# chiy48308/audio_feature_extraction

Measured on AMD Instinct MI355X. Metric: audio frames/sec (sr=22050, n_fft=1024, hop=256, n_mfcc=13), higher is better.
Workload: dtype f32; 1 GPU; 1000x10s clips @22050 Hz per GPU, frame_length=1024, hop_length=256, n_mfcc=13, n_mels=128, hamming, pre-emphasis 0.97 + trim 30 dB + RMS (BASELINE configs[1]); clips_per_gpu=1000, frames_per_gpu_step=862000, input=HBM-resident float32

## Files before the change

### audio_feature_extraction_amd/csrc/afx_api.cpp

```cpp
#include <algorithm>
#include <cmath>
#include <cstdio>
#include <cstdlib>
#include <cstring>
#include <atomic>
#include <mutex>
#include <string>
#include <vector>

#include <hip/hip_runtime.h>

#include "afx_device.h"
#include "afx_devenv.h"
#include "afx_frames3.h"
#include "afx_internal.h"
#include "afx_plan.h"

namespace afx {
DevEnv::DevEnv() {
  if (const char* v = getenv("AFX_DEBUG_SKIP")) debug_skip = atoi(v) & 127;
  if (const char* v = getenv("AFX_F0_DEBUG")) f0_debug = atoi(v);
  stamps = getenv("AFX_DEBUG_STAMPS") != nullptr;
  f3_debug = getenv("AFX_F3_DEBUG") != nullptr;
  no_spec = getenv("AFX_NO_SPEC") != nullptr;
  no_tickets = getenv("AFX_NO_TICKETS") != nullptr;
  no_frames3 = getenv("AFX_NO_FRAMES3") != nullptr;
  no_frames3s = getenv("AFX_NO_FRAMES3S") != nullptr;
  no_frames3d = getenv("AFX_NO_FRAMES3D") != nullptr;
  f3_generic_mel = getenv("AFX_F3_GENERIC_MEL") != nullptr;
  no_dct16l = getenv("AFX_NO_DCT16L") != nullptr;
  host_blocks = getenv("AFX_HOST_BLOCKS") != nullptr;
  no_fused_tail = getenv("AFX_NO_FUSED_TAIL") != nullptr;
  if (const char* v = getenv("AFX_F3_WAVES")) f3_waves = atoi(v);
  if (const char* v = getenv("AFX_F3_SPARE_CUS")) f3_spare_cus = atoi(v) < 0 ? -2 : atoi(v);
  if (const char* v = getenv("AFX_TAIL_MODE")) tail_mode = atoi(v);
  if (const char* v = getenv("AFX_TAIL_SKIP")) tail_skip = atoi(v) & 7;
  if (const char* v = getenv("AFX_TEST_CHUNK_CLIPS")) chunk_clips = std::max(1, std::min(32768, atoi(v)));
  if (const char* v = getenv("AFX_TEST_F0_CHUNK_FRAMES")) f0_chunk_frames = std::max<int64_t>(64, atoll(v));
  if (const char* v = getenv("AFX_TEST_DTW_BUDGET")) dtw_budget = std::max<int64_t>(1, atoll(v));
  if (const char* v = getenv("AFX_TEST_HPSS_BUDGET")) hpss_budget = std::max<int64_t>(1, atoll(v));
  if (const char* v = getenv("AFX_TEST_CHROMA_BUDGET")) chroma_budget = std::max<int64_t>(1, atoll(v));
  if (const char* v = getenv("AFX_TEST_RHYTHM_BUDGET")) rhythm_budget = std::max<int64_t>(1, atoll(v));
  if (const char* v = getenv("AFX_TEST_GROUPS_BUDGET")) groups_budget = std::max<int64_t>(1, atoll(v));
  if (const char* v = getenv("AFX_TEST_FILT_BUDGET")) filt_budget = std::max<int64_t>(1, atoll(v));
  f0_dump = getenv("AFX_F0_DUMP");
}
const DevEnv& dev_env() { static const DevEnv e; return e; }
}

extern "C" int afx_device_count(void) {
  int n = 0;
  if (hipGetDeviceCount(&n) != hipSuccess) return 0;
  return n;
}

extern "C" int afx_init(int device, afx_ctx** out) {
  if (!out) { set_error("afx_init: null out"); return AFX_ERR_INVALID; }
  *out = nullptr;
  int n = afx_device_count();
  if (n <= 0) { set_error("no HIP device visible"); return AFX_ERR_NO_DEVICE; }
  if (device < 0 || device >= n) { set_error("device index out of range"); return AFX_ERR_INVALID; }
  HIP_TRY(hipSetDevice(device));
  afx_ctx* c = new afx_ctx();
  c->device = device;
  hipError_t e = hipStreamCreateWithFlags(&c->stream, hipStreamNonBlocking);
  if (e != hipSuccess) { delete c; set_error(std::string("hipStreamCreate: ") + hipGetErrorString(e)); return AFX_ERR_HIP; }
  *out = c;
  return AFX_OK;
}

extern "C" void afx_destroy(afx_ctx* ctx) {
  if (!ctx) return;
  (void)hipSetDevice(ctx->device);
  for (DevBuf* b : {&ctx->dtw_raw, &ctx->dtw_feats, &ctx->dtw_norms, &ctx->dtw_pairs, &ctx->dtw_codes, &ctx->dtw_rows, &ctx->dtw_d,
                    &ctx->dtw_path, &ctx->dtw_cost, &ctx->dtw_status, &ctx->dtw_len, &ctx->dtw_end, &ctx->rs_g, &ctx->rs_tstart, &ctx->rs_clips,
                    &ctx->rs_in, &ctx->rs_out, &ctx->dc_clips, &ctx->dc_in, &ctx->dc_out, &ctx->ft_tab, &ctx->ft_clips, &ctx->ft_st,
                    &ctx->ft_w, &ctx->ft_carry, &ctx->ft_tmax, &ctx->ft_in, &ctx->ft_out})
    release(*b);
  if (ctx->stream) (void)hipStreamDestroy(ctx->stream);
  delete ctx;
}

extern "C" int afx_malloc(afx_ctx* ctx, size_t bytes, void** out) {
  if (!ctx || !out) { set_error("afx_malloc: null argument"); return AFX_ERR_INVALID; }
  HIP_TRY(hipSetDevice(ctx->device));
  hipError_t e = hipMalloc(out, bytes ? bytes : 1);
  if (e != hipSuccess) { set_error(std::string("hipMalloc: ") + hipGetErrorString(e)); return e == hipErrorOutOfMemory ? AFX_ERR_NOMEM : AFX_ERR_HIP; }
  return AFX_OK;
}

extern "C" int afx_free(afx_ctx* ctx, void* d) {
  if (!ctx) { set_error("afx_free: null ctx"); return AFX_ERR_INVALID; }
  HIP_TRY(hipSetDevice(ctx->device));
  if (d) HIP_TRY(hipFree(d));
  return AFX_OK;
}

extern "C" int afx_host_alloc(afx_ctx* ctx, size_t bytes, void** out) {
  if (!ctx || !out) { set_error("afx_host_alloc: null argument"); return AFX_ERR_INVALID; }
  *out = nullptr;
  HIP_TRY(hipSetDevice(ctx->device));
  hipError_t e = hipHostMalloc(out, bytes ? bytes : 1, hipHostMallocPortable);
  if (e != hipSuccess) { set_error(std::string("hipHostMalloc: ") + hipGetErrorString(e)); *out = nullptr; return e == hipErrorOutOfMemory ? AFX_ERR_NOMEM : AFX_ERR_HIP; }
  return AFX_OK;
}

extern "C" int afx_host_free(afx_ctx* ctx, void* h) {
  if (!ctx) { set_error("afx_host_free: null ctx"); return AFX_ERR_INVALID; }
  HIP_TRY(hipSetDevice(ctx->device));
  if (h) HIP_TRY(hipHostFree(h));
  return AFX_OK;
}

extern "C" int afx_memcpy_h2d(afx_ctx* ctx, void* dst, const void* src, size_t bytes) {
  if (!ctx || (!dst && bytes) || (!src && bytes)) { set_error("afx_memcpy_h2d: null argument"); return AFX_ERR_INVALID; }
  HIP_TRY(hipSetDevice(ctx->device));
  HIP_TRY(hipMemcpyAsync(dst, src, bytes, hipMemcpyHostToDevice, ctx->stream));
  HIP_TRY(hipStreamSynchronize(ctx->stream));
  return AFX_OK;
}

extern "C" int afx_memcpy_d2h(afx_ctx* ctx, void* dst, const void* src, size_t bytes) {
  if (!ctx || (!dst && bytes) || (!src && bytes)) { set_error("afx_memcpy_d2h: null argument"); return AFX_ERR_INVALID; }
  HIP_TRY(hipSetDevice(ctx->device));
  HIP_TRY(hipMemcpyAsync(dst, src, bytes, hipMemcpyDeviceToHost, ctx->stream));
  HIP_TRY(hipStreamSynchronize(ctx->stream));
  return AFX_OK;
}

extern "C" int afx_synchronize(afx_ctx* ctx) {
  if (!ctx) { set_error("afx_synchronize: null ctx"); return AFX_ERR_INVALID; }
  HIP_TRY(hipSetDevice(ctx->device));
  HIP_TRY(hipStreamSynchronize(ctx->stream));
  return AFX_OK;
}

template <typename T>
static int upload(afx_plan* pl, const T* host, size_t count, const T** dev) {
  void* d = nullptr;
  size_t bytes = std::max<size_t>(count * sizeof(T), 16);
  hipError_t e = hipMalloc(&d, bytes);
  if (e != hipSuccess) { set_error(std::string("hipMalloc(table): ") + hipGetErrorString(e)); return AFX_ERR_HIP; }
  pl->table_allocs.push_back(d);
  HIP_TRY(hipMemset(d, 0, bytes));
  if (count) HIP_TRY(hipMemcpy(d, host, count * sizeof(T), hipMemcpyHostToDevice));
  *dev = (const T*)d;
  return AFX_OK;
}

static std::mutex g_submitted_mu;
static std::vector<std::pair<int, hipStream_t>> g_submitted;
static bool other_stream_in_flight(int device, hipStream_t s) {
  std::lock_guard<std::mutex> lk(g_submitted_mu);
  for (const auto& e : g_submitted) if (e.first == device && e.second != s) return true;
  return false;
}
static void list_submitted(afx_plan* pl, hipStream_t s) {
  std::lock_guard<std::mutex> lk(g_submitted_mu);
  g_submitted.emplace_back(pl->device, s);
  pl->pend.listed = true; pl->pend.stream = s;
}
static void unlist_submitted(afx_plan* pl) {
  if (!pl->pend.listed) return;
  pl->pend.listed = false;
  std::lock_guard<std::mutex> lk(g_submitted_mu);
  const auto it = std::find(g_submitted.begin(), g_submitted.end(), std::make_pair(pl->device, pl->pend.stream));
  if (it != g_submitted.end()) g_submitted.erase(it);
}

extern "C" int afx_plan_create(afx_ctx* ctx, const afx_params* p, afx_plan** out) {
  if (!ctx || !p || !out) { set_error("afx_plan_create: null argument"); return AFX_ERR_INVALID; }
  *out = nullptr;
  std::string msg;
  int st = validate_params(*p, msg);
  if (st != AFX_OK) { set_error(msg); return st; }
  if (p->n_fft > 2048) { set_error("frame_length > 2048 is not supported by the LDS-resident FFT"); return AFX_ERR_UNSUPPORTED; }
  HIP_TRY(hipSetDevice(ctx->device));
  afx_plan* pl = new afx_plan();
  pl->ctx = ctx; pl->device = ctx->device; pl->p = *p;
  build_host_tables(*p, pl->ht);
  const size_t lds = frames_mr_shape(p->n_fft) ? frames_mr_lds_bytes(p->n_fft, p->hop) : frames_lds_bytes(p->n_fft, p->hop);
  if (lds == 0 || lds > 160 * 1024) {
// ... 620 lines not shown
```

### audio_feature_extraction_amd/csrc/afx_devenv.h

```cpp
#pragma once
#include <cstdint>

namespace afx {

struct DevEnv {
  int debug_skip = 0, f0_debug = 0;
  bool stamps = false, f3_debug = false, no_spec = false, no_tickets = false;
  bool no_frames3 = false, no_frames3s = false, no_frames3d = false;
  bool f3_generic_mel = false;
  bool no_dct16l = false;
  bool host_blocks = false;
  bool no_fused_tail = false;
  int tail_mode = 0;
  int tail_skip = 0;
  int f3_waves = 0;
  int f3_spare_cus = -1;
  int chunk_clips = 32768;
  int64_t f0_chunk_frames = 1280 * 1024;
  int64_t dtw_budget = (int64_t)2 << 30;
  int64_t hpss_budget = (int64_t)2 << 30;
  int64_t chroma_budget = (int64_t)2 << 30;
  int64_t rhythm_budget = (int64_t)2 << 30;
  int64_t groups_budget = (int64_t)2 << 30;
  int64_t filt_budget = (int64_t)2 << 30;
  const char* f0_dump = nullptr;
  DevEnv();
};
const DevEnv& dev_env();

}
```

### audio_feature_extraction_amd/csrc/afx_frames3.hip

```cpp
#include <hip/hip_runtime.h>

#include <algorithm>
#include <cstdlib>
#include <type_traits>

#include "afx_device.h"
#include "afx_devenv.h"
#include "afx_frames3.h"
#include "afx_frames3_dev.h"

namespace afx {

size_t frames3_lds_bytes(int waves, const F3Tables& ft) {
  return (size_t)(waves * kF3ExFloats + kF3TabFloats + ft.mel_wfloats + ft.mel_rounds * 64 + 1024) * sizeof(float);
}

#ifdef AFX_F3_DEBUG
__device__ unsigned long long g_f3_stamps[4 * 8192];
__device__ unsigned long long g_f3_blk[65536];
#endif

template <int FMT, int WAVES, int NB0, int NB1, bool SPEC>
__global__ __launch_bounds__(WAVES * 64) void k_frames3(const void* __restrict__ samples,
                                                        ClipInfo* __restrict__ info,
                                                        const BlockDesc* __restrict__ blocks, int nblocks,
                                                        const int* __restrict__ nblocks_dev,
                                                        F3Tables ft, KParams kp,
                                                        float* __restrict__ logmel,
                                                        float* __restrict__ blockmax,
                                                        float* __restrict__ bsum,
                                                        int* __restrict__ work_ctr) {
  constexpr int N = 1024, HOP = 256;
  extern __shared__ __attribute__((aligned(16))) float smem[];
  if (nblocks_dev) {
    nblocks = *nblocks_dev;
    if (nblocks <= 0) return;
  }
  const int tid = threadIdx.x, lane = tid & 63;
  const int wave = __builtin_amdgcn_readfirstlane(tid >> 6);
#ifdef AFX_F3_DEBUG
  const unsigned long long stamp0 = wall_clock64();
#endif
  float* const tabs = smem + WAVES * kF3ExFloats;
  float4* const T2q = reinterpret_cast<float4*>(tabs);
  float4* const T3q = reinterpret_cast<float4*>(tabs + 256);
  const int mel_wfloats = NB0 > 0 ? (NB0 + NB1) * 256 : ft.mel_wfloats;
  const int mel_rounds = NB0 > 0 ? 2 : ft.mel_rounds;
  float* const MW = tabs + kF3TabFloats;
  int* const MM = reinterpret_cast<int*>(MW + mel_wfloats);
  v2* const E = reinterpret_cast<v2*>(smem + wave * kF3ExFloats);
  float* const XB = reinterpret_cast<float*>(E);

  {
    const v2* w1024 = reinterpret_cast<const v2*>(ft.w1024);
    auto W = [&](int m) { const v2 v = w1024[m & 511]; return (m & 512) ? -v : v; };
    if (tid < 64) {
      const int rr = tid >> 4, c = tid & 15;
      const v2 a = W(8 * (2 * rr) * c), b = W(8 * (2 * rr + 1) * c);
      T2q[tid] = float4{a.x, a.y, b.x, b.y};
      const int jbt = tid ? 128 - tid : 64;
#pragma unroll
      for (int r = 1; r < 8; ++r) { const v2 ta = W(tid * r), tb = W(jbt * r); T3q[(r - 1) * 64 + tid] = float4{ta.x, ta.y, tb.x, tb.y}; }
    }
    for (int i = tid; i < mel_wfloats; i += WAVES * 64) MW[i] = ft.mel_w[i];
    for (int i = tid; i < mel_rounds * 64; i += WAVES * 64) MM[i] = ft.mel_meta[i];
    for (int i = lane; i < kF3ExFloats; i += 64) XB[i] = 0.f;
  }
  float4* const WT = reinterpret_cast<float4*>(MM + mel_rounds * 64);
  if (tid < 64) {
    float wreg[16];
#pragma unroll
    for (int u = 0; u < 16; ++u) wreg[u] = 0.5f * ft.window[u < 8 ? lane + 64 * u : (64 - lane) + 64 * (15 - u)];
#pragma unroll
    for (int v = 0; v < 4; ++v) WT[v * 64 + lane] = float4{wreg[4 * v], wreg[4 * v + 1], wreg[4 * v + 2], wreg[4 * v + 3]};
  }
  __syncthreads();
  const v2 H = {0.70710678118654752440f, 0.70710678118654752440f};
  const v2 W1 = {0.92387953251128675613f, -0.38268343236508977173f};
  const v2 W3 = {0.38268343236508977173f, -0.92387953251128675613f};
  const bool pre = (kp.flags & AFX_FLAG_PREEMPH) != 0;
  const float b1 = pre ? kp.preemph_b1 : 0.f;
  const int M = kp.n_mels;
  const int jb = lane ? 128 - lane : 64;
  v2* const e1w = E + lane;
  const v2* const e1r = E + 66 * (lane & 15) + (lane >> 4);
  v2* const e2w = E + 128 * (lane >> 4) + (lane & 15);
  v2* const ea = E + lane;
  v2* const eb = E + jb;

  using sample_t = sample_of<FMT>;
  const int n_rounds = mel_rounds;
  const int meta0 = MM[lane], meta1 = MM[64 + lane];
  const unsigned mf0 = (meta0 >> 11) & 511, mf1 = (meta1 >> 11) & 511;
  const float amin = kp.amin;

  float bs = 0.f;
  unsigned long long bsmask = 0;
  auto sub2 = [&](float x, float y, int idx, unsigned long long two) -> bool {
    const float m = f3_sum2(x, y);
    const unsigned long long sel = two << idx;
    bs = f3_sel(bs, m, sel);
    bsmask |= sel;
    return __any(!(fabsf(m) < INFINITY));
  };
  auto flag_nonfinite = [&](const BlockDesc& bd, bool bad_rows) {
    if (__any(bad_rows) && lane == 0) atomicOr(&info[bd.clip].nonfinite, 1u);
  };
  auto sub_store = [&](const BlockDesc& bd) {
    const int j = bd.t0 + lane;
    if (((bsmask >> lane) & 1) && j < bd.bsum_n) bsum[bd.bsum_base + j] = bs;
    bsmask = 0;
  };

  const int total_waves = gridDim.x * WAVES, wg = blockIdx.x * WAVES + wave;
#ifdef AFX_F3_DEBUG
  const unsigned long long stamp1 = wall_clock64();
#endif
  F3Runs runs = f3_runs_init(work_ctr, nblocks, total_waves, wg, true);
  do {
  const int b_hi = runs.b_hi;
  for (int b = runs.b_lo; b < b_hi; ++b) {
    BlockDesc bd = blocks[b];
    if (!bd.active) continue;
    bool first = true;
    v2 Ra[8], Rb[8];
    for (;;) {
    const int Tleft = bd.T - bd.t0;
    const int npairs = Tleft >= 16 ? 8 : (Tleft + 1) >> 1;
    bool chain = false;
    if (SPEC && npairs == 8 && b + 1 < b_hi) {
      const BlockDesc* nx = blocks + b + 1;
      chain = nx->active && nx->clip == bd.clip && nx->t0 == bd.t0 + 16;
    }
    const int64_t sbase = bd.sample_base;
    const sample_t* const sp = (const sample_t*)samples + sbase;
    auto interior = [&](int j0, int j1) -> bool {
      return (j0 - 1 >= bd.have_lo) && (j1 <= bd.have_hi) && (j0 >= bd.keep_lo) && (j1 <= bd.keep_hi);
    };
    auto interior_r = [&](int j0, int j1) -> bool {
      const BlockDesc& r = blocks[f3_opaque(b)];
      return (j0 - 1 >= r.have_lo) && (j1 <= r.have_hi) && (j0 >= r.keep_lo) && (j1 <= r.keep_hi);
    };
    auto edge_sample = [&](int j) -> float {
      const BlockDesc& bd = blocks[f3_opaque(b)];
      const int lo = bd.have_lo, hi = bd.have_hi - 1;
      const int jc = j < lo ? lo : (j > hi ? hi : j), jp = (j - 1) < lo ? lo : ((j - 1) > hi ? hi : (j - 1));
      const float y = (jc == j) ? ld_raw<FMT>(samples, sbase + jc) : 0.f;
      const float yp = (jp == j - 1) ? ld_raw<FMT>(samples, sbase + jp) : 0.f;
      float v = y;
      if (pre) {
        v = preemph1(y, yp, b1);
        if (j == lo) v = preemph0(ld_raw<FMT>(samples, bd.clip_off), ld_raw<FMT>(samples, bd.clip_off + 1));
      }
      return (j >= bd.keep_lo && j < bd.keep_hi) ? v : 0.f;
    };

    if (first) {
      float rows[20];
      if (interior(0, N + HOP)) {
        float y[20], yp[20];
#pragma unroll
        for (int u = 0; u < 20; ++u) { y[u] = ld_row<FMT>(sp, 64 * u + lane); yp[u] = ld_row<FMT>(sp - 1, 64 * u + lane); }
#pragma unroll
        for (int u = 0; u < 20; ++u) rows[u] = preemph1(y[u], yp[u], b1);
      } else {
#pragma unroll 1
        for (int u = 0; u < 20; ++u) XB[64 * u + lane] = edge_sample(64 * u + lane);
#pragma unroll
        for (int u = 0; u < 20; ++u) rows[u] = XB[64 * u + lane];
      }
#pragma unroll
      for (int u = 0; u < 8; ++u) { Ra[u] = v2{rows[u], rows[u + 4]}; Rb[u] = v2{rows[u + 8], rows[u + 12]}; }
      if constexpr (SPEC) {
        auto sq4 = [&](int r) { float q = rows[r] * rows[r]; q = fmaf(rows[r + 1], rows[r + 1], q); q = fmaf(rows[r + 2], rows[r + 2], q); return fmaf(rows[r + 3], rows[r + 3], q); };
        auto bad4 = [&](int r) { return !(isfinite(rows[r]) && isfinite(rows[r + 1]) && isfinite(rows[r + 2]) && isfinite(rows[r + 3])); };
        if (sub2(sq4(12), sq4(16), 1, 3ull)) flag_nonfinite(bd, bad4(12) || bad4(16));
        if (bd.t0 == 0 && sub2(0.f, sq4(8), 0, 1ull)) flag_nonfinite(bd, bad4(8));
      }
    }
    float lmax = -INFINITY;
    float* const tile = logmel + bd.frame_slot * (int64_t)M;
    const bool blk_int = interior(0, 512 * 8 + 768 + 512);

    auto pair_body = [&](v2 (&P)[8], v2 (&Q)[8], const int p) __attribute__((always_inline)) {
      v2 z[16];
#pragma unroll
      for (int v = 0; v < 4; ++v) {
        const float4 w = ldv4(WT + v * 64 + lane);
        const v2* const src = v < 2 ? P + 4 * v : Q + 4 * (v - 2);
        z[4 * v] = src[0] * v2{w.x, w.x}; z[4 * v + 1] = src[1] * v2{w.y, w.y};
        z[4 * v + 2] = src[2] * v2{w.z, w.z}; z[4 * v + 3] = src[3] * v2{w.w, w.w};
      }
      const bool more = p + 1 < npairs || chain;
      const int jn = 512 * (p + 1) + 768;
      const bool nint = more && (blk_int || interior_r(jn, jn + 512));

      f3_dft16(z, H, W1, W3);
      if (!F3_SKIP(0x200)) {
#pragma unroll
      for (int k = 0; k < 16; ++k) stv(e1w + 66 * k, z[k]);
#pragma unroll
      for (int u = 0; u < 16; ++u) z[u] = ldv(e1r + 4 * u);
      }
      {
        v2 tw[8];
#pragma unroll
        for (int rr = 0; rr < 4; ++rr) {
          const float4 t = ldv4(T2q + rr * 16 + (lane & 15));
          tw[2 * rr] = v2{t.x, t.y}; tw[2 * rr + 1] = v2{t.z, t.w};
        }
        v2 xa[8], xb[8];
#pragma unroll
        for (int r = 0; r < 8; ++r) { xa[r] = z[2 * r]; xb[r] = z[2 * r + 1]; }
#pragma unroll
        for (int r = 1; r < 8; ++r) cmul2(xa[r], tw[r], xb[r], tw[r]);
        f3_dft8(xa, H); f3_dft8(xb, H);
        if (!F3_SKIP(0x2000)) {
#pragma unroll
        for (int r = 0; r < 8; ++r) { stv(e2w + 16 * r, xa[r]); stv(e2w + 16 * r + 512, xb[r]); }
        } else {
#pragma unroll
          for (int r = 0; r < 8; ++r) { z[2 * r] = xa[r]; z[2 * r + 1] = xb[r]; }
        }
      }
      v2 A[8], B[8];
      if (!F3_SKIP(0x2000)) {
#pragma unroll
      for (int r = 0; r < 8; ++r) { A[r] = ldv(ea + 128 * r); B[r] = ldv(eb + 128 * r); }
      } else {
#pragma unroll
        for (int r = 0; r < 8; ++r) { A[r] = z[r]; B[r] = z[r + 8]; }
      }
#pragma unroll
      for (int r = 1; r < 8; ++r) {
        const float4 t = ldv4(T3q + (r - 1) * 64 + lane);
        cmul2(A[r], v2{t.x, t.y}, B[r], v2{t.z, t.w});
      }
      f3_dft8(A, H); f3_dft8(B, H);
      v2 nyq = A[4];
      if (lane == 0) { A[4] = B[4]; B[4] = A[5]; A[5] = B[5]; B[5] = A[6]; A[6] = B[6]; B[6] = A[7]; A[7] = B[7]; B[7] = A[0]; }
      if (!F3_SKIP(0x800)) {
#pragma unroll
      for (int s = 0; s < 4; s += 2) {
        v2 p0, p1;
        sqsum2(A[s] + B[7 - s], A[s] - B[7 - s], A[s + 1] + B[6 - s], A[s + 1] - B[6 - s], p0, p1);
        ea[128 * s] = p0; ea[128 * (s + 1)] = p1;
      }
#pragma unroll
      for (int s = 4; s < 8; s += 2) {
        v2 p0, p1;
        sqsum2(A[s] + B[7 - s], A[s] - B[7 - s], A[s + 1] + B[6 - s], A[s + 1] - B[6 - s], p0, p1);
        eb[384 - 128 * (s - 4)] = p0; eb[384 - 128 * (s - 3)] = p1;
      }
      if (lane == 0) E[512] = v2{4.f * nyq.x * nyq.x, 4.f * nyq.y * nyq.y};
      } else {
        asm volatile("" :: "v"(A[0]), "v"(A[1]), "v"(A[2]), "v"(A[3]), "v"(A[4]), "v"(A[5]), "v"(A[6]), "v"(A[7]));
        asm volatile("" :: "v"(B[0]), "v"(B[1]), "v"(B[2]), "v"(B[3]), "v"(B[4]), "v"(B[5]), "v"(B[6]), "v"(B[7]), "v"(nyq));
      }

      float ny[8], nyp[8];
      if (nint) {
#pragma unroll
        for (int u = 0; u < 8; ++u) { ny[u] = ld_row<FMT>(sp + jn, 64 * u + lane); nyp[u] = ld_row<FMT>(sp + jn - 1, 64 * u + lane); }
      }
      __builtin_amdgcn_s_setprio(1);
      const bool vA = 2 * p < Tleft, vB = 2 * p + 1 < Tleft;
      float* const rowA = tile + (unsigned)(2 * p * M);
      if constexpr (NB0 > 0) {
        if (!F3_SKIP(0x400)) {
        const float4* pp0 = reinterpret_cast<const float4*>(E + (meta0 & 2047));
        const float4* pp1 = reinterpret_cast<const float4*>(E + (meta1 & 2047));
        const float4* ww0 = reinterpret_cast<const float4*>(MW) + lane;
        const float4* ww1 = reinterpret_cast<const float4*>(MW + NB0 * 256) + lane;
        v2 s0[4], s1[4];
#pragma unroll
        for (int i = 0; i < NB0; ++i) {
          const float4 c = ww0[64 * i], q0 = pp0[2 * i], q1 = pp0[2 * i + 1];
          const v2 c01 = {c.x, c.y}, c23 = {c.z, c.w};
          if (i == 0) {
            s0[0] = f3_mel_mul_lo(v2{q0.x, q0.y}, c01); s0[1] = f3_mel_mul_hi(v2{q0.z, q0.w}, c01);
            s0[2] = f3_mel_mul_lo(v2{q1.x, q1.y}, c23); s0[3] = f3_mel_mul_hi(v2{q1.z, q1.w}, c23);
          } else {
            s0[0] = f3_mel_fma_lo(v2{q0.x, q0.y}, c01, s0[0]); s0[1] = f3_mel_fma_hi(v2{q0.z, q0.w}, c01, s0[1]);
            s0[2] = f3_mel_fma_lo(v2{q1.x, q1.y}, c23, s0[2]); s0[3] = f3_mel_fma_hi(v2{q1.z, q1.w}, c23, s0[3]);
          }
        }
#pragma unroll
        for (int i = 0; i < NB1; ++i) {
          const float4 c = ww1[64 * i], q0 = pp1[2 * i], q1 = pp1[2 * i + 1];
          const v2 c01 = {c.x, c.y}, c23 = {c.z, c.w};
          if (i == 0) {
            s1[0] = f3_mel_mul_lo(v2{q0.x, q0.y}, c01); s1[1] = f3_mel_mul_hi(v2{q0.z, q0.w}, c01);
            s1[2] = f3_mel_mul_lo(v2{q1.x, q1.y}, c23); s1[3] = f3_mel_mul_hi(v2{q1.z, q1.w}, c23);
          } else {
            s1[0] = f3_mel_fma_lo(v2{q0.x, q0.y}, c01, s1[0]); s1[1] = f3_mel_fma_hi(v2{q0.z, q0.w}, c01, s1[1]);
            s1[2] = f3_mel_fma_lo(v2{q1.x, q1.y}, c23, s1[2]); s1[3] = f3_mel_fma_hi(v2{q1.z, q1.w}, c23, s1[3]);
          }
        }
        const v2 m0 = (s0[0] + s0[1]) + (s0[2] + s0[3]), m1 = (s1[0] + s1[1]) + (s1[2] + s1[3]);
        const float L00 = 3.01029995663981195f * __builtin_amdgcn_logf(f3_max(m0.x, amin));
        const float L01 = 3.01029995663981195f * __builtin_amdgcn_logf(f3_max(m0.y, amin));
        const float L10 = 3.01029995663981195f * __builtin_amdgcn_logf(f3_max(m1.x, amin));
        const float L11 = 3.01029995663981195f * __builtin_amdgcn_logf(f3_max(m1.y, amin));
        rowA[mf0] = L00; rowA[mf1] = L10;
        lmax = f3_max(lmax, f3_max(L00, L10));
        if (vB) {
          rowA[M + mf0] = L01; rowA[M + mf1] = L11;
          lmax = f3_max(lmax, f3_max(L01, L11));
        }
        }
      } else {
#pragma unroll 1
      for (int rd = 0; rd < (F3_SKIP(0x400) ? 0 : n_rounds); ++rd) {
        const uint32_t rp = ft.mel_rp[rd];
        const int meta = MM[rd * 64 + lane];
        const float4* pp = reinterpret_cast<const float4*>(E + (meta & 2047));
        const float4* ww = reinterpret_cast<const float4*>(MW + (rp >> 8)) + lane;
        const int nb = rp & 15, wd = (rp >> 4) & 15;
        v2 a0 = {0.f, 0.f}, a1 = {0.f, 0.f};
#define F3_BATCH(i)                                                                  \
        if (nb > (i)) {                                                              \
          const float4 c = ww[64 * (i)];                                             \
          const float4 q0 = pp[2 * (i)], q1 = pp[2 * (i) + 1];                       \
          a0 = v2{q0.x, q0.y} * v2{c.x, c.x} + a0; a1 = v2{q0.z, q0.w} * v2{c.y, c.y} + a1; \
          a0 = v2{q1.x, q1.y} * v2{c.z, c.z} + a0; a1 = v2{q1.z, q1.w} * v2{c.w, c.w} + a1; \
        }
        F3_BATCH(0) F3_BATCH(1) F3_BATCH(2) F3_BATCH(3) F3_BATCH(4) F3_BATCH(5) F3_BATCH(6) F3_BATCH(7)
#undef F3_BATCH
        v2 acc = a0 + a1;
        if (wd >= 2) { acc.x += AFX_DPP_F(acc.x, 0xB1, false); acc.y += AFX_DPP_F(acc.y, 0xB1, false); }
        if (wd >= 4) { acc.x += AFX_DPP_F(acc.x, 0x4E, false); acc.y += AFX_DPP_F(acc.y, 0x4E, false); }
        if (wd >= 8) { acc.x += AFX_DPP_F(acc.x, 0x141, false); acc.y += AFX_DPP_F(acc.y, 0x141, false); }
        const float L0 = 3.01029995663981195f * __builtin_amdgcn_logf(f3_max(acc.x, amin));
        const float L1 = 3.01029995663981195f * __builtin_amdgcn_logf(f3_max(acc.y, amin));
        if (meta & (1 << 20)) {
          const unsigned m = (meta >> 11) & 511;
          if (vA) rowA[m] = L0;
          if (vB) rowA[M + m] = L1;
          if (vA) lmax = f3_max(lmax, L0);
          if (vB) lmax = f3_max(lmax, L1);
        }
      }
      }

      __builtin_amdgcn_s_setprio(0);
      if (more) {
        float n[8];
        if (nint) {
#pragma unroll
          for (int u = 0; u < 8; ++u) n[u] = preemph1(ny[u], nyp[u], b1);
        } else {
          const int jn_e = f3_opaque(jn);
#pragma unroll 1
          for (int u = 0; u < 8; ++u) XB[64 * u + lane] = edge_sample(jn_e + 64 * u + lane);
#pragma unroll
          for (int u = 0; u < 8; ++u) n[u] = XB[64 * u + lane];
        }
#pragma unroll
        for (int i = 0; i < 4; ++i) { P[i] = v2{Q[4 + i].y, n[i]}; P[4 + i] = v2{n[i], n[4 + i]}; }
        if constexpr (SPEC) {
          v2 q = P[4] * P[4]; q = P[5] * P[5] + q; q = P[6] * P[6] + q; q = P[7] * P[7] + q;
          if (sub2(q.x, q.y, 2 * p + 3, 3ull)) {
            bool bad = false;
#pragma unroll
            for (int u = 0; u < 8; ++u) bad |= !isfinite(n[u]);
            flag_nonfinite(blocks[f3_opaque(b)], bad);
          }
        }
      }
    };

#pragma unroll 1
    for (int p = 0; p < npairs; p += 2) {
      pair_body(Ra, Rb, p);
      if (p + 1 < npairs) pair_body(Rb, Ra, p + 1);
    }
    {
      const float mx = f3_wave_max(lmax);
      const BlockDesc& be = blocks[f3_opaque(b)];
      if constexpr (SPEC) { if (lane == 0) blockmax[b] = mx; sub_store(be); }
      else { if (lane == 0 && mx > -INFINITY) atomicMax(&info[be.clip].lmax_ord, f2ord(mx)); }
    }
#ifdef AFX_F3_DEBUG
    if (SPEC && lane == 0 && b < 65536) g_f3_blk[b] = wall_clock64();
#endif
    if (!chain) break;
    first = false;
    ++b;
    bd = blocks[b];
    }
  }
  } while (f3_runs_next(runs, work_ctr, nblocks, (int)(gridDim.x * WAVES), lane));
#ifdef AFX_F3_DEBUG
  if (SPEC && lane == 0 && wg < 8192) {
    g_f3_stamps[4 * wg] = stamp0; g_f3_stamps[4 * wg + 1] = stamp1; g_f3_stamps[4 * wg + 2] = wall_clock64();
    g_f3_stamps[4 * wg + 3] = (unsigned long long)__builtin_amdgcn_s_getreg((31 << 11) | 4) |
                              ((unsigned long long)__builtin_amdgcn_s_getreg((31 << 11) | 20) << 32);
  }
#endif
}

#ifdef AFX_F3_DEBUG
extern "C" __attribute__((visibility("default"))) int afx_debug_f3_stamps(unsigned long long* out, int n_waves) {
  return (int)hipMemcpyFromSymbol(out, HIP_SYMBOL(g_f3_stamps), sizeof(unsigned long long) * 4 * (size_t)n_waves);
}
extern "C" __attribute__((visibility("default"))) int afx_debug_f3_blocks(unsigned long long* out, int n_blocks) {
  return (int)hipMemcpyFromSymbol(out, HIP_SYMBOL(g_f3_blk), sizeof(unsigned long long) * (size_t)n_blocks);
}
#endif

bool frames3_eligible(const KParams& kp, const F3Tables& ft) {
  const int per = kp.hop > 0 ? kp.trim_hop / kp.hop : 0;
  if (!(ft.mel_rounds > 0 && kp.n_mels <= 512 && kp.hop > 0 && kp.trim_hop % kp.hop == 0 && per >= 1 && per <= 4) ||
      dev_env().no_frames3)
    return false;
  if (kp.n_fft == 1024 && kp.hop == 256) return frames3_lds_bytes(12, ft) <= 160 * 1024;
  if (kp.n_fft == 2048 && kp.hop == 512) return frames3s_lds_bytes(12, ft) <= 160 * 1024 && !dev_env().no_frames3s;
  if (kp.n_fft == 512 && kp.hop == 128) return frames3d_lds_bytes(12, ft) <= 160 * 1024 && !dev_env().no_frames3d;
  return false;
}

hipError_t launch_frames3_any(const F3Launch& L) {
  if (L.kp.n_fft == 2048) return launch_frames3s(L);
  if (L.kp.n_fft == 512) return launch_frames3d(L);
  return launch_frames3(L);
}

int frames3_waves(const F3Tables& ft) {
  const int forced = dev_env().f3_waves;
  if (forced == 12 || forced == 16) return frames3_lds_bytes(forced, ft) <= 160 * 1024 ? forced : 12;
  return frames3_lds_bytes(16, ft) <= 160 * 1024 ? 16 : 12;
}

int f3_spare_cus(const KParams& kp, int nblocks, int n_cu, bool other_in_flight) {
  const int forced = dev_env().f3_spare_cus;
  if (forced >= 0) return forced;
  if (!other_in_flight || nblocks < 2 * 16 * n_cu) return 0;
  const int r = ((kp.n_fft == 1024 && kp.hop == 256) || (kp.n_fft == 512 && kp.hop == 128)) ? 64 : 0;
  return std::min(r, n_cu / 4 / kF3Xcds * kF3Xcds);
}

template <int FMT, int WAVES, int NB0, int NB1, bool SPEC>
static hipError_t launch_frames3_t(const F3Launch& L) {
  const hipError_t e = allow_lds_once<k_frames3<FMT, WAVES, NB0, NB1, SPEC>>();
  if (e != hipSuccess) return e;
  hipLaunchKernelGGL((k_frames3<FMT, WAVES, NB0, NB1, SPEC>), dim3(f3_grid(L, WAVES)), dim3(WAVES * 64), frames3_lds_bytes(WAVES, L.ft), L.s,
                     L.samples, L.info, L.blocks, L.nblocks, L.nblocks_dev, L.ft, L.kp, L.logmel, L.blockmax, L.bsum, L.work_ctr);
  return hipGetLastError();
}

template <int FMT, int WAVES, bool SPEC>
static hipError_t launch_frames3_w(const F3Launch& L) {
  const F3Tables& ft = L.ft;
  const bool two = ft.mel_rounds == 2 && ((ft.mel_rp[0] >> 4) & 15) == 1 && ((ft.mel_rp[1] >> 4) & 15) == 1 && ft.mel_all_own &&
                   ft.mel_wfloats == (int)((ft.mel_rp[0] & 15) + (ft.mel_rp[1] & 15)) * 256 && (ft.mel_rp[1] >> 8) == (ft.mel_rp[0] & 15) * 256 &&
                   !dev_env().f3_generic_mel;
  const int nb0 = ft.mel_rp[0] & 15, nb1 = ft.mel_rp[1] & 15;
  if (two && nb0 == 2 && nb1 == 7)
    return launch_frames3_t<FMT, WAVES, 2, 7, SPEC>(L);
  return launch_frames3_t<FMT, WAVES, 0, 0, SPEC>(L);
}

hipError_t launch_frames3(const F3Launch& L) {
  const int waves = frames3_waves(L.ft);
#define AFX_F3_GO(FMT, W) (L.spec ? launch_frames3_w<FMT, W, true>(L) : launch_frames3_w<FMT, W, false>(L))
  if (L.kp.fmt == AFX_FMT_S16) return waves == 16 ? AFX_F3_GO(AFX_FMT_S16, 16) : AFX_F3_GO(AFX_FMT_S16, 12);
  return waves == 16 ? AFX_F3_GO(AFX_FMT_F32, 16) : AFX_F3_GO(AFX_FMT_F32, 12);
#undef AFX_F3_GO
}

}
```

### audio_feature_extraction_amd/csrc/afx_frames3_dev.h

```cpp
#pragma once
#include <hip/hip_runtime.h>

#include <cstdint>

#include "afx_device.h"
#include "afx_frames3.h"
#include "afx_wave.h"

namespace afx {

typedef float v2 __attribute__((ext_vector_type(2)));

__device__ __forceinline__ v2 add_mi(v2 a, v2 b) {
  v2 d; asm("v_pk_add_f32 %0, %1, %2 op_sel:[0,1] op_sel_hi:[1,0] neg_hi:[0,1]" : "=v"(d) : "v"(a), "v"(b)); return d;
}
__device__ __forceinline__ v2 add_pi(v2 a, v2 b) {
  v2 d; asm("v_pk_add_f32 %0, %1, %2 op_sel:[0,1] op_sel_hi:[1,0] neg_lo:[0,1]" : "=v"(d) : "v"(a), "v"(b)); return d;
}
__device__ __forceinline__ v2 cmul(v2 v, v2 w) {
  v2 t, d;
  asm("v_pk_mul_f32 %0, %1, %2 op_sel_hi:[1,0]" : "=v"(t) : "v"(v), "v"(w));
  asm("v_pk_fma_f32 %0, %1, %2, %3 op_sel:[1,1,0] op_sel_hi:[0,1,1] neg_lo:[1,0,0]" : "=v"(d) : "v"(v), "v"(w), "v"(t));
  return d;
}
__device__ __forceinline__ void cmul2(v2& a, v2 wa, v2& b, v2 wb) {
  v2 ta, tb, da, db;
  asm("v_pk_mul_f32 %0, %1, %2 op_sel_hi:[1,0]" : "=v"(ta) : "v"(a), "v"(wa));
  asm("v_pk_mul_f32 %0, %1, %2 op_sel_hi:[1,0]" : "=v"(tb) : "v"(b), "v"(wb));
  asm("v_pk_fma_f32 %0, %1, %2, %3 op_sel:[1,1,0] op_sel_hi:[0,1,1] neg_lo:[1,0,0]" : "=v"(da) : "v"(a), "v"(wa), "v"(ta));
  asm("v_pk_fma_f32 %0, %1, %2, %3 op_sel:[1,1,0] op_sel_hi:[0,1,1] neg_lo:[1,0,0]" : "=v"(db) : "v"(b), "v"(wb), "v"(tb));
  a = da; b = db;
}
__device__ __forceinline__ v2 cmul_s(v2 v, v2 w) {
  v2 t, d;
  asm("v_pk_mul_f32 %0, %1, %2 op_sel_hi:[1,0]" : "=v"(t) : "v"(v), "s"(w));
  asm("v_pk_fma_f32 %0, %1, %2, %3 op_sel:[1,1,0] op_sel_hi:[0,1,1] neg_lo:[1,0,0]" : "=v"(d) : "v"(v), "s"(w), "v"(t));
  return d;
}
__device__ __forceinline__ void cmul2_s(v2& a, v2 wa, v2& b, v2 wb) {
  v2 ta, tb, da, db;
  asm("v_pk_mul_f32 %0, %1, %2 op_sel_hi:[1,0]" : "=v"(ta) : "v"(a), "s"(wa));
  asm("v_pk_mul_f32 %0, %1, %2 op_sel_hi:[1,0]" : "=v"(tb) : "v"(b), "s"(wb));
  asm("v_pk_fma_f32 %0, %1, %2, %3 op_sel:[1,1,0] op_sel_hi:[0,1,1] neg_lo:[1,0,0]" : "=v"(da) : "v"(a), "s"(wa), "v"(ta));
  asm("v_pk_fma_f32 %0, %1, %2, %3 op_sel:[1,1,0] op_sel_hi:[0,1,1] neg_lo:[1,0,0]" : "=v"(db) : "v"(b), "s"(wb), "v"(tb));
  a = da; b = db;
}
__device__ __forceinline__ v2 fma_mi(v2 e, v2 H, v2 b) {
  v2 d; asm("v_pk_fma_f32 %0, %1, %2, %3 op_sel:[1,0,0] op_sel_hi:[0,0,1] neg_hi:[1,0,0]" : "=v"(d) : "v"(e), "s"(H), "v"(b)); return d;
}
__device__ __forceinline__ v2 fma_pi(v2 e, v2 H, v2 b) {
  v2 d; asm("v_pk_fma_f32 %0, %1, %2, %3 op_sel:[1,0,0] op_sel_hi:[0,0,1] neg_lo:[1,0,0]" : "=v"(d) : "v"(e), "s"(H), "v"(b)); return d;
}
__device__ __forceinline__ v2 sqsum(v2 s, v2 d) {
  v2 t, r;
  asm("v_pk_mul_f32 %0, %1, %1" : "=v"(t) : "v"(s));
  asm("v_pk_fma_f32 %0, %1, %1, %2 op_sel:[1,1,0] op_sel_hi:[0,0,1]" : "=v"(r) : "v"(d), "v"(t));
  return r;
}

__device__ __forceinline__ void sqsum2(v2 s0, v2 d0, v2 s1, v2 d1, v2& r0, v2& r1) {
  v2 t0, t1;
  asm("v_pk_mul_f32 %0, %1, %1" : "=v"(t0) : "v"(s0));
  asm("v_pk_mul_f32 %0, %1, %1" : "=v"(t1) : "v"(s1));
  asm("v_pk_fma_f32 %0, %1, %1, %2 op_sel:[1,1,0] op_sel_hi:[0,0,1]" : "=v"(r0) : "v"(d0), "v"(t0));
  asm("v_pk_fma_f32 %0, %1, %1, %2 op_sel:[1,1,0] op_sel_hi:[0,0,1]" : "=v"(r1) : "v"(d1), "v"(t1));
}
__device__ __forceinline__ float f3_max(float a, float b) {
  float r; asm("v_max_f32 %0, %1, %2" : "=v"(r) : "v"(a), "v"(b)); return r;
}

typedef const volatile v2 __attribute__((address_space(3))) * f3_lds_cv2;
__device__ __forceinline__ v2 ldv(const v2* p) { return *(f3_lds_cv2)(p); }
typedef volatile v2 __attribute__((address_space(3))) * f3_lds_v2;
__device__ __forceinline__ void stv(v2* p, v2 v) { *(f3_lds_v2)(p) = v; }
typedef const volatile float4 __attribute__((address_space(3))) * f3_lds_cv4;
__device__ __forceinline__ float4 ldv4(const float4* p) {
  const float __attribute__((ext_vector_type(4))) v = *(const volatile float __attribute__((ext_vector_type(4))) __attribute__((address_space(3)))*)(p);
  return float4{v.x, v.y, v.z, v.w};
}

__device__ __forceinline__ v2 f3_mel_mul_lo(v2 q, v2 c) {
  v2 d; asm("v_pk_mul_f32 %0, %1, %2 op_sel_hi:[1,0]" : "=v"(d) : "v"(q), "v"(c)); return d;
}
__device__ __forceinline__ v2 f3_mel_mul_hi(v2 q, v2 c) {
  v2 d; asm("v_pk_mul_f32 %0, %1, %2 op_sel:[0,1] op_sel_hi:[1,1]" : "=v"(d) : "v"(q), "v"(c)); return d;
}
__device__ __forceinline__ v2 f3_mel_fma_lo(v2 q, v2 c, v2 a) {
  v2 d; asm("v_pk_fma_f32 %0, %1, %2, %3 op_sel_hi:[1,0,1]" : "=v"(d) : "v"(q), "v"(c), "v"(a)); return d;
}
__device__ __forceinline__ v2 f3_mel_fma_hi(v2 q, v2 c, v2 a) {
  v2 d; asm("v_pk_fma_f32 %0, %1, %2, %3 op_sel:[0,1,0] op_sel_hi:[1,1,1]" : "=v"(d) : "v"(q), "v"(c), "v"(a)); return d;
}

__device__ __forceinline__ void f3_dft4(v2& x0, v2& x1, v2& x2, v2& x3) {
  const v2 a = x0 + x2, b = x0 - x2, c = x1 + x3, e = x1 - x3;
  x0 = a + c; x2 = a - c; x1 = add_mi(b, e); x3 = add_pi(b, e);
}

__device__ __forceinline__ void f3_dft8(v2* x, const v2 H) {
  v2 e0 = x[0], e1 = x[2], e2 = x[4], e3 = x[6];
  v2 o0 = x[1], o1 = x[3], o2 = x[5], o3 = x[7];
  f3_dft4(e0, e1, e2, e3);
  f3_dft4(o0, o1, o2, o3);
  const v2 q1 = add_mi(o1, o1);
  const v2 q3 = add_pi(o3, o3);
  x[0] = e0 + o0; x[4] = e0 - o0;
  x[1] = q1 * H + e1; x[5] = e1 - q1 * H;
  x[2] = add_mi(e2, o2); x[6] = add_pi(e2, o2);
  x[3] = e3 - q3 * H; x[7] = q3 * H + e3;
}

__device__ __forceinline__ void f3_dft16(v2* x, const v2 H, const v2 W1, const v2 W3) {
  v2 t0[4], t1[4], t2[4], t3[4];
#pragma unroll
  for (int n2 = 0; n2 < 4; ++n2) {
    v2 a = x[n2], b = x[n2 + 4], c = x[n2 + 8], d = x[n2 + 12];
    f3_dft4(a, b, c, d);
    t0[n2] = a; t1[n2] = b; t2[n2] = c; t3[n2] = d;
  }
  {
    f3_dft4(t0[0], t0[1], t0[2], t0[3]);
    x[0] = t0[0]; x[4] = t0[1]; x[8] = t0[2]; x[12] = t0[3];
  }
  {
    v2 p1 = t1[1], p3 = t1[3];
    cmul2_s(p1, W1, p3, W3);
    const v2 q = add_mi(t1[2], t1[2]);
    const v2 a = q * H + t1[0], b = t1[0] - q * H, c = p1 + p3, e = p1 - p3;
    x[1] = a + c; x[9] = a - c; x[5] = add_mi(b, e); x[13] = add_pi(b, e);
  }
  {
    const v2 q1 = add_mi(t2[1], t2[1]), q3 = add_pi(t2[3], t2[3]);
    const v2 a = add_mi(t2[0], t2[2]), b = add_pi(t2[0], t2[2]);
    const v2 c = q1 - q3, e = q1 + q3;
    x[2] = c * H + a; x[10] = a - c * H; x[6] = fma_mi(e, H, b); x[14] = fma_pi(e, H, b);
  }
  {
    v2 p1 = t3[1], m3 = t3[3];
    cmul2_s(p1, W3, m3, W1);
    const v2 q = add_pi(t3[2], t3[2]);
    const v2 a = t3[0] - q * H, b = q * H + t3[0], c = p1 - m3, e = p1 + m3;
    x[3] = a + c; x[11] = a - c; x[7] = add_mi(b, e); x[15] = add_pi(b, e);
  }
}

__device__ __forceinline__ int f3_opaque(int x) { asm volatile("" : "+s"(x)); return x; }
#ifdef AFX_F3_DEBUG
#define F3_SKIP(bit) ((kp.flags & (bit)) != 0)
#else
#define F3_SKIP(bit) false
#endif
struct F3Runs {
  int b_lo, b_hi, stride;
};
__device__ __forceinline__ F3Runs f3_runs_init(const int* work_ctr, int nblocks, int total_waves, int wg, bool contiguous) {
  F3Runs r;
  r.stride = 1;
  if (work_ctr) {
    const int C0 = nblocks / (2 * total_waves);
    r.b_lo = wg * C0; r.b_hi = r.b_lo + C0;
  } else if (contiguous) {
    r.b_lo = (int)((long long)wg * nblocks / total_waves); r.b_hi = (int)((long long)(wg + 1) * nblocks / total_waves);
  } else {
    r.b_lo = wg; r.b_hi = nblocks; r.stride = total_waves;
  }
  return r;
}
__device__ __forceinline__ bool f3_runs_next(F3Runs& r, int* work_ctr, int nblocks, int total_waves, int lane) {
  if (!work_ctr) return false;
  int t = 0;
  if (lane == 0) t = atomicAdd(work_ctr, 1);
  t = __builtin_amdgcn_readfirstlane(t);
  const int C0 = nblocks / (2 * total_waves), dyn0 = total_waves * C0;
  const int cA = C0 / 2 > 1 ? C0 / 2 : 1, cB = C0 / 3 > 1 ? C0 / 3 : 1;
  int c = 1;
  if (t < total_waves) { r.b_lo = dyn0 + cA * t; c = cA; }
  else if (t < 2 * total_waves) { r.b_lo = dyn0 + cA * total_waves + cB * (t - total_waves); c = cB; }
  else r.b_lo = dyn0 + (cA + cB) * total_waves + (t - 2 * total_waves);
  if (r.b_lo >= nblocks) return false;
  r.b_hi = r.b_lo + c < nblocks ? r.b_lo + c : nblocks;
  return true;
}

__device__ __forceinline__ float f3_add_xor16(float v) {
  const auto r = __builtin_amdgcn_permlane16_swap(__float_as_uint(v), __float_as_uint(v), false, false);
  return __uint_as_float(r[0]) + __uint_as_float(r[1]);
}
__device__ __forceinline__ float f3_add_xor32(float v) {
  const auto r = __builtin_amdgcn_permlane32_swap(__float_as_uint(v), __float_as_uint(v), false, false);
  return __uint_as_float(r[0]) + __uint_as_float(r[1]);
}
__device__ __forceinline__ float f3_sel(float a, float b, unsigned long long mask) {
  float d; asm("v_cndmask_b32_e64 %0, %1, %2, %3" : "=v"(d) : "v"(a), "v"(b), "s"(mask)); return d;
}
__device__ __forceinline__ float f3_sum2(float x, float y) {
  x += AFX_DPP_F(x, 0xB1, false); y += AFX_DPP_F(y, 0xB1, false);
  float m = f3_sel(y, x, 0xAAAAAAAAAAAAAAAAull);
  m += AFX_DPP_F(m, 0x4E, false);
  m += AFX_DPP_F(m, 0x124, false); m += AFX_DPP_F(m, 0x128, false);
  return f3_add_xor32(f3_add_xor16(m));
}

template <int FMT>
__device__ __forceinline__ float f3_edge_sample(const void* samples, const BlockDesc& bd, int64_t sbase, bool pre, float b1, int j) {
  const int lo = bd.have_lo, hi = bd.have_hi - 1;
  const int jc = j < lo ? lo : (j > hi ? hi : j), jp = (j - 1) < lo ? lo : ((j - 1) > hi ? hi : (j - 1));
  const float y = (jc == j) ? ld_raw<FMT>(samples, sbase + jc) : 0.f;
  const float yp = (jp == j - 1) ? ld_raw<FMT>(samples, sbase + jp) : 0.f;
  float v = y;
  if (pre) {
    v = preemph1(y, yp, b1);
    if (j == lo) v = preemph0(ld_raw<FMT>(samples, bd.clip_off), ld_raw<FMT>(samples, bd.clip_off + 1));
  }
  return (j >= bd.keep_lo && j < bd.keep_hi) ? v : 0.f;
}
struct F3Max { __device__ float operator()(float a, float b) const { return f3_max(a, b); } };
__device__ __forceinline__ float f3_wave_max(float v) {
  v = row_reduce(v, F3Max());
  return fmaxf(fmaxf(row_total(v, 0), row_total(v, 1)), fmaxf(row_total(v, 2), row_total(v, 3)));
}

}
```

Baseline: 1.346 billion frames/s.

## Software-pipeline LDS twiddle and mel-weight reads with explicit lgkmcnt waits

Adds a PIPE template variant of the frames3 kernel, enabled by default for the compiled-in 2+7 mel schedule. It issues ds_read_b128 loads for the FFT twiddle tables (T2, T3), the window and the mel weights/spectra several stages ahead through inline asm. It then waits with precise s_waitcnt lgkmcnt counts, so LDS latency overlaps the complex multiplies and FMAs instead of stalling on each load. It also fuses the spectrum square-accumulate into packed FMAs. The cost is more live VGPRs for the prefetched values and fragile hand-counted waitcnt values, which are wrong if the compiler reorders or inserts LDS operations.

```diff
diff --git a/audio_feature_extraction_amd/csrc/afx_api.cpp b/audio_feature_extraction_amd/csrc/afx_api.cpp
--- a/audio_feature_extraction_amd/csrc/afx_api.cpp
+++ b/audio_feature_extraction_amd/csrc/afx_api.cpp
@@ -28,6 +28,7 @@
   no_frames3s = getenv("AFX_NO_FRAMES3S") != nullptr;
   no_frames3d = getenv("AFX_NO_FRAMES3D") != nullptr;
   f3_generic_mel = getenv("AFX_F3_GENERIC_MEL") != nullptr;
+  if (const char* v = getenv("AFX_F3_LDS_PIPE")) f3_lds_pipe = atoi(v) != 0;
   no_dct16l = getenv("AFX_NO_DCT16L") != nullptr;
   host_blocks = getenv("AFX_HOST_BLOCKS") != nullptr;
   no_fused_tail = getenv("AFX_NO_FUSED_TAIL") != nullptr;
diff --git a/audio_feature_extraction_amd/csrc/afx_devenv.h b/audio_feature_extraction_amd/csrc/afx_devenv.h
--- a/audio_feature_extraction_amd/csrc/afx_devenv.h
+++ b/audio_feature_extraction_amd/csrc/afx_devenv.h
@@ -8,6 +8,7 @@
   bool stamps = false, f3_debug = false, no_spec = false, no_tickets = false;
   bool no_frames3 = false, no_frames3s = false, no_frames3d = false;
   bool f3_generic_mel = false;
+  bool f3_lds_pipe = true;
   bool no_dct16l = false;
   bool host_blocks = false;
   bool no_fused_tail = false;
diff --git a/audio_feature_extraction_amd/csrc/afx_frames3.hip b/audio_feature_extraction_amd/csrc/afx_frames3.hip
--- a/audio_feature_extraction_amd/csrc/afx_frames3.hip
+++ b/audio_feature_extraction_amd/csrc/afx_frames3.hip
@@ -15,12 +15,15 @@
   return (size_t)(waves * kF3ExFloats + kF3TabFloats + ft.mel_wfloats + ft.mel_rounds * 64 + 1024) * sizeof(float);
 }
 
+constexpr int kF3MelDepth = 2;
+constexpr int kF3T3Depth = 5;
+
 #ifdef AFX_F3_DEBUG
 __device__ unsigned long long g_f3_stamps[4 * 8192];
 __device__ unsigned long long g_f3_blk[65536];
 #endif
 
-template <int FMT, int WAVES, int NB0, int NB1, bool SPEC>
+template <int FMT, int WAVES, int NB0, int NB1, bool SPEC, bool PIPE>
 __global__ __launch_bounds__(WAVES * 64) void k_frames3(const void* __restrict__ samples,
                                                         ClipInfo* __restrict__ info,
                                                         const BlockDesc* __restrict__ blocks, int nblocks,
@@ -30,6 +33,7 @@
                                                         float* __restrict__ blockmax,
                                                         float* __restrict__ bsum,
                                                         int* __restrict__ work_ctr) {
+  static_assert(!PIPE || NB0 > 0, "the pipelined LDS reads belong to the compiled-in mel schedule");
   constexpr int N = 1024, HOP = 256;
   extern __shared__ __attribute__((aligned(16))) float smem[];
   if (nblocks_dev) {
@@ -82,6 +86,11 @@
   const float b1 = pre ? kp.preemph_b1 : 0.f;
   const int M = kp.n_mels;
   const int jb = lane ? 128 - lane : 64;
+  constexpr int kT3Off = 256 * 4, kMWOff = kF3TabFloats * 4, kWTOff = (kF3TabFloats + (NB0 + NB1) * 256 + 2 * 64) * 4;
+  unsigned LT2 = f3_lds_addr(smem) + (unsigned)(WAVES * kF3ExFloats) * 4 + 16 * (lane & 15);
+  unsigned LB = f3_lds_addr(smem) + (unsigned)(WAVES * kF3ExFloats) * 4 + 16 * lane;
+  const unsigned LE = f3_lds_addr(smem) + (unsigned)(wave * kF3ExFloats) * 4;
+  if constexpr (PIPE) asm volatile("" : "+v"(LT2), "+v"(LB));
   v2* const e1w = E + lane;
   const v2* const e1r = E + 66 * (lane & 15) + (lane >> 4);
   v2* const e2w = E + 128 * (lane >> 4) + (lane & 15);
@@ -186,7 +195,14 @@
       v2 z[16];
 #pragma unroll
       for (int v = 0; v < 4; ++v) {
-        const float4 w = ldv4(WT + v * 64 + lane);
+        float4 w;
+        if constexpr (PIPE) {
+          const v4 t = v == 0 ? f3_lds_ld128<kWTOff>(LB) : v == 1 ? f3_lds_ld128<kWTOff + 1024>(LB)
+                     : v == 2 ? f3_lds_ld128<kWTOff + 2048>(LB) : f3_lds_ld128<kWTOff + 3072>(LB);
+          w = float4{t.x, t.y, t.z, t.w};
+        } else {
+          w = ldv4(WT + v * 64 + lane);
+        }
         const v2* const src = v < 2 ? P + 4 * v : Q + 4 * (v - 2);
         z[4 * v] = src[0] * v2{w.x, w.x}; z[4 * v + 1] = src[1] * v2{w.y, w.y};
         z[4 * v + 2] = src[2] * v2{w.z, w.z}; z[4 * v + 3] = src[3] * v2{w.w, w.w};
@@ -196,24 +212,43 @@
       const bool nint = more && (blk_int || interior_r(jn, jn + 512));
 
       f3_dft16(z, H, W1, W3);
+      v4 t2[4];
       if (!F3_SKIP(0x200)) {
 #pragma unroll
       for (int k = 0; k < 16; ++k) stv(e1w + 66 * k, z[k]);
+      if constexpr (PIPE) {
+        f3_static_for<0, 4>([&](auto rr) {
+#pragma unroll
+          for (int u = 4 * rr; u < 4 * rr + 4; ++u) z[u] = ldv(e1r + 4 * u);
+          f3_lds_rd128<256 * rr>(t2[rr], LT2);
+        });
+      } else {
 #pragma unroll
       for (int u = 0; u < 16; ++u) z[u] = ldv(e1r + 4 * u);
       }
+      } else if constexpr (PIPE) {
+        f3_static_for<0, 4>([&](auto rr) { f3_lds_rd128<256 * rr>(t2[rr], LT2); });
+      }
       {
+        v2 xa[8], xb[8];
+#pragma unroll
+        for (int r = 0; r < 8; ++r) { xa[r] = z[2 * r]; xb[r] = z[2 * r + 1]; }
+        if constexpr (PIPE) {
+          f3_static_for<0, 4>([&](auto rr) {
+            if (!F3_SKIP(0x200)) f3_lds_wait<5 * (3 - rr)>(t2[rr]); else f3_lds_wait<3 - rr>(t2[rr]);
+            if constexpr (rr > 0) cmul2(xa[2 * rr], t2[rr].xy, xb[2 * rr], t2[rr].xy);
+            cmul2(xa[2 * rr + 1], t2[rr].zw, xb[2 * rr + 1], t2[rr].zw);
+          });
+        } else {
         v2 tw[8];
 #pragma unroll
         for (int rr = 0; rr < 4; ++rr) {
           const float4 t = ldv4(T2q + rr * 16 + (lane & 15));
           tw[2 * rr] = v2{t.x, t.y}; tw[2 * rr + 1] = v2{t.z, t.w};
         }
-        v2 xa[8], xb[8];
-#pragma unroll
-        for (int r = 0; r < 8; ++r) { xa[r] = z[2 * r]; xb[r] = z[2 * r + 1]; }
 #pragma unroll
         for (int r = 1; r < 8; ++r) cmul2(xa[r], tw[r], xb[r], tw[r]);
+        }
         f3_dft8(xa, H); f3_dft8(xb, H);
         if (!F3_SKIP(0x2000)) {
 #pragma unroll
@@ -231,10 +266,22 @@
 #pragma unroll
         for (int r = 0; r < 8; ++r) { A[r] = z[r]; B[r] = z[r + 8]; }
       }
+      if constexpr (PIPE) {
+        v4 t3[7];
+        constexpr int D3 = kF3T3Depth;
+        auto issue3 = [&](auto k) { f3_lds_rd128<kT3Off + 1024 * k>(t3[k], LB); };
+        f3_static_for<0, D3>(issue3);
+        f3_static_for<0, 7>([&](auto k) {
+          f3_lds_wait<(k + D3 < 7 ? k + D3 : 7) - (k + 1)>(t3[k]);
+          cmul2(A[k + 1], t3[k].xy, B[k + 1], t3[k].zw);
+          if constexpr (k + D3 < 7) issue3(std::integral_constant<int, k + D3>{});
+        });
+      } else {
 #pragma unroll
       for (int r = 1; r < 8; ++r) {
         const float4 t = ldv4(T3q + (r - 1) * 64 + lane);
         cmul2(A[r], v2{t.x, t.y}, B[r], v2{t.z, t.w});
+      }
       }
       f3_dft8(A, H); f3_dft8(B, H);
       v2 nyq = A[4];
@@ -273,6 +320,32 @@
         const float4* ww0 = reinterpret_cast<const float4*>(MW) + lane;
         const float4* ww1 = reinterpret_cast<const float4*>(MW + NB0 * 256) + lane;
         v2 s0[4], s1[4];
+        if constexpr (PIPE) {
+          constexpr int NB = NB0 + NB1, D = kF3MelDepth;
+          const unsigned pa0 = LE + 8 * (meta0 & 2047), pa1 = LE + 8 * (meta1 & 2047);
+          v4 rc[NB], rq0[NB], rq1[NB];
+          auto issue = [&](auto b) {
+            constexpr int i = b;
+            f3_lds_rd128<kMWOff + 1024 * i>(rc[i], LB);
+            if constexpr (i < NB0) { f3_lds_rd128<32 * i>(rq0[i], pa0); f3_lds_rd128<32 * i + 16>(rq1[i], pa0); }
+            else { f3_lds_rd128<32 * (i - NB0)>(rq0[i], pa1); f3_lds_rd128<32 * (i - NB0) + 16>(rq1[i], pa1); }
+          };
+          f3_static_for<0, (D < NB ? D : NB)>(issue);
+          f3_static_for<0, NB>([&](auto b) {
+            constexpr int i = b;
+            f3_lds_wait<3 * ((i + D < NB ? i + D : NB) - (i + 1))>(rc[i], rq0[i], rq1[i]);
+            const v2 c01 = rc[i].xy, c23 = rc[i].zw;
+            v2* const s = i < NB0 ? s0 : s1;
+            if constexpr (i == 0 || i == NB0) {
+              s[0] = f3_mel_mul_lo(rq0[i].xy, c01); s[1] = f3_mel_mul_hi(rq0[i].zw, c01);
+              s[2] = f3_mel_mul_lo(rq1[i].xy, c23); s[3] = f3_mel_mul_hi(rq1[i].zw, c23);
+            } else {
+              s[0] = f3_mel_fma_lo(rq0[i].xy, c01, s[0]); s[1] = f3_mel_fma_hi(rq0[i].zw, c01, s[1]);
+              s[2] = f3_mel_fma_lo(rq1[i].xy, c23, s[2]); s[3] = f3_mel_fma_hi(rq1[i].zw, c23, s[3]);
+            }
+            if constexpr (i + D < NB) issue(std::integral_constant<int, i + D>{});
+          });
+        } else {
 #pragma unroll
         for (int i = 0; i < NB0; ++i) {
           const float4 c = ww0[64 * i], q0 = pp0[2 * i], q1 = pp0[2 * i + 1];
@@ -296,6 +369,7 @@
             s1[0] = f3_mel_fma_lo(v2{q0.x, q0.y}, c01, s1[0]); s1[1] = f3_mel_fma_hi(v2{q0.z, q0.w}, c01, s1[1]);
             s1[2] = f3_mel_fma_lo(v2{q1.x, q1.y}, c23, s1[2]); s1[3] = f3_mel_fma_hi(v2{q1.z, q1.w}, c23, s1[3]);
           }
+        }
         }
         const v2 m0 = (s0[0] + s0[1]) + (s0[2] + s0[3]), m1 = (s1[0] + s1[1]) + (s1[2] + s1[3]);
         const float L00 = 3.01029995663981195f * __builtin_amdgcn_logf(f3_max(m0.x, amin));
@@ -359,7 +433,12 @@
 #pragma unroll
         for (int i = 0; i < 4; ++i) { P[i] = v2{Q[4 + i].y, n[i]}; P[4 + i] = v2{n[i], n[4 + i]}; }
         if constexpr (SPEC) {
-          v2 q = P[4] * P[4]; q = P[5] * P[5] + q; q = P[6] * P[6] + q; q = P[7] * P[7] + q;
+          v2 q = P[4] * P[4];
+          if constexpr (PIPE) {
+            q = f3_sq_acc(P[5], q); q = f3_sq_acc(P[6], q); q = f3_sq_acc(P[7], q);
+          } else {
+            q = P[5] * P[5] + q; q = P[6] * P[6] + q; q = P[7] * P[7] + q;
+          }
           if (sub2(q.x, q.y, 2 * p + 3, 3ull)) {
             bool bad = false;
 #pragma unroll
@@ -440,11 +519,11 @@
   return std::min(r, n_cu / 4 / kF3Xcds * kF3Xcds);
 }
 
-template <int FMT, int WAVES, int NB0, int NB1, bool SPEC>
+template <int FMT, int WAVES, int NB0, int NB1, bool SPEC, bool PIPE>
 static hipError_t launch_frames3_t(const F3Launch& L) {
-  const hipError_t e = allow_lds_once<k_frames3<FMT, WAVES, NB0, NB1, SPEC>>();
+  const hipError_t e = allow_lds_once<k_frames3<FMT, WAVES, NB0, NB1, SPEC, PIPE>>();
   if (e != hipSuccess) return e;
-  hipLaunchKernelGGL((k_frames3<FMT, WAVES, NB0, NB1, SPEC>), dim3(f3_grid(L, WAVES)), dim3(WAVES * 64), frames3_lds_bytes(WAVES, L.ft), L.s,
+  hipLaunchKernelGGL((k_frames3<FMT, WAVES, NB0, NB1, SPEC, PIPE>), dim3(f3_grid(L, WAVES)), dim3(WAVES * 64), frames3_lds_bytes(WAVES, L.ft), L.s,
                      L.samples, L.info, L.blocks, L.nblocks, L.nblocks_dev, L.ft, L.kp, L.logmel, L.blockmax, L.bsum, L.work_ctr);
   return hipGetLastError();
 }
@@ -457,8 +536,8 @@
                    !dev_env().f3_generic_mel;
   const int nb0 = ft.mel_rp[0] & 15, nb1 = ft.mel_rp[1] & 15;
   if (two && nb0 == 2 && nb1 == 7)
-    return launch_frames3_t<FMT, WAVES, 2, 7, SPEC>(L);
-  return launch_frames3_t<FMT, WAVES, 0, 0, SPEC>(L);
+    return dev_env().f3_lds_pipe ? launch_frames3_t<FMT, WAVES, 2, 7, SPEC, true>(L) : launch_frames3_t<FMT, WAVES, 2, 7, SPEC, false>(L);
+  return launch_frames3_t<FMT, WAVES, 0, 0, SPEC, false>(L);
 }
 
 hipError_t launch_frames3(const F3Launch& L) {
diff --git a/audio_feature_extraction_amd/csrc/afx_frames3_dev.h b/audio_feature_extraction_amd/csrc/afx_frames3_dev.h
--- a/audio_feature_extraction_amd/csrc/afx_frames3_dev.h
+++ b/audio_feature_extraction_amd/csrc/afx_frames3_dev.h
@@ -2,6 +2,7 @@
 #include <hip/hip_runtime.h>
 
 #include <cstdint>
+#include <type_traits>
 
 #include "afx_device.h"
 #include "afx_frames3.h"
@@ -56,6 +57,10 @@
   asm("v_pk_mul_f32 %0, %1, %1" : "=v"(t) : "v"(s));
   asm("v_pk_fma_f32 %0, %1, %1, %2 op_sel:[1,1,0] op_sel_hi:[0,0,1]" : "=v"(r) : "v"(d), "v"(t));
   return r;
+}
+
+__device__ __forceinline__ v2 f3_sq_acc(v2 x, v2 a) {
+  v2 d; asm("v_pk_fma_f32 %0, %1, %1, %2" : "=v"(d) : "v"(x), "v"(a)); return d;
 }
 
 __device__ __forceinline__ void sqsum2(v2 s0, v2 d0, v2 s1, v2 d1, v2& r0, v2& r1) {
@@ -77,6 +82,34 @@
 __device__ __forceinline__ float4 ldv4(const float4* p) {
   const float __attribute__((ext_vector_type(4))) v = *(const volatile float __attribute__((ext_vector_type(4))) __attribute__((address_space(3)))*)(p);
   return float4{v.x, v.y, v.z, v.w};
+}
+
+typedef float v4 __attribute__((ext_vector_type(4)));
+__device__ __forceinline__ unsigned f3_lds_addr(const void* p) {
+  return (unsigned)(uintptr_t)(const __attribute__((address_space(3))) void*)p;
+}
+template <int OFF>
+__device__ __forceinline__ void f3_lds_rd128(v4& d, unsigned addr) {
+  static_assert(OFF >= 0 && OFF < 65536 && OFF % 16 == 0, "ds offset");
+  asm volatile("ds_read_b128 %0, %1 offset:%2" : "=v"(d) : "v"(addr), "i"(OFF) : "memory");
+}
+template <int N>
+__device__ __forceinline__ void f3_lds_wait(v4& a) {
+  static_assert(N >= 0, "operations issued behind the one waited for");
+  asm volatile("s_waitcnt lgkmcnt(%1)" : "+v"(a) : "i"(N < 15 ? N : 14));
+}
+template <int N>
+__device__ __forceinline__ void f3_lds_wait(v4& a, v4& b, v4& c) {
+  static_assert(N >= 0, "operations issued behind the one waited for");
+  asm volatile("s_waitcnt lgkmcnt(%3)" : "+v"(a), "+v"(b), "+v"(c) : "i"(N < 15 ? N : 14));
+}
+template <int OFF>
+__device__ __forceinline__ v4 f3_lds_ld128(unsigned addr) {
+  return *(const volatile v4 __attribute__((address_space(3)))*)(uintptr_t)(addr + OFF);
+}
+template <int LO, int HI, class F>
+__device__ __forceinline__ void f3_static_for(F&& f) {
+  if constexpr (LO < HI) { f(std::integral_constant<int, LO>{}); f3_static_for<LO + 1, HI>(f); }
 }
 
 __device__ __forceinline__ v2 f3_mel_mul_lo(v2 q, v2 c) {
```

Result: no change. 1.341 billion frames/s, median of 2 (-0.4%).
